# vineetbansal/scarlet

Hardware: AMD Instinct MI355X
Metric: PGM iters/sec on 10k 5-band 64x64 scenes (higher is better)
Workload: dtype f32

## Files before the change

include/scarlet_hip.h:

```cpp
#ifndef SCARLET_HIP_H
#define SCARLET_HIP_H

#include <stdint.h>

#ifdef __cplusplus
extern "C" {
#endif

#define SCARLET_OK            0
#define SCARLET_E_ARG        -1
#define SCARLET_E_TOO_LARGE  -2
#define SCARLET_E_HIP        -3
#define SCARLET_E_NOTIMPL    -4

#define SCARLET_MAX_SIDE     1024
#define SCARLET_MAX_COMPONENTS 256
#define SCARLET_MAX_OBSERVATIONS 8

#define SCARLET_FLAG_SED_NOT_CONVERGED   1
#define SCARLET_FLAG_MORPH_NOT_CONVERGED 2
#define SCARLET_FLAG_EDGE_PIXELS         4
#define SCARLET_FLAG_NO_VALID_PIXELS     8

#define SCARLET_STATUS_CENTER_AT_EDGE    1
#define SCARLET_STATUS_NONFINITE         2
#define SCARLET_STATUS_BAD_COUNT         4
#define SCARLET_STATUS_BAD_INIT          8

#define SCARLET_INIT_EXTENDED 0
#define SCARLET_INIT_POINT    1
#define SCARLET_MAX_LAYERS    8

#define SCARLET_SYM_KSPACE 0
#define SCARLET_SYM_SOFT   1
#define SCARLET_SYM_SDSS   2
#define SCARLET_SYM_FULL_WINDOW 16

#define SCARLET_NORM_SED       0
#define SCARLET_NORM_MORPH     1
#define SCARLET_NORM_MORPH_MAX 2

const char *scarlet_version(void);
const char *scarlet_last_error(void);
int scarlet_set_option(const char *name, int value);
int64_t scarlet_debug_stamps(int64_t *out, int64_t capacity);
int scarlet_next_fast_len(int n);


int scarlet_host_prox_monotonic_f64(double *x, int n, const int *ref_idx,
                                    const int *dist_idx, int n_dist, double thresh);

int scarlet_host_prox_weighted_monotonic_f32(float *x, int n, const float *weights,
                                             const int *offsets, const int *dist_idx,
                                             int n_dist, float thresh);
int scarlet_host_prox_weighted_monotonic_f64(double *x, int n, const double *weights,
                                             const int *offsets, const int *dist_idx,
                                             int n_dist, double thresh);

int scarlet_host_apply_filter_f32(const float *image, int H, int W, const float *values,
                                  const int *y_start, const int *y_end, const int *x_start,
                                  const int *x_end, int n, float *result);
int scarlet_host_apply_filter_f64(const double *image, int H, int W, const double *values,
                                  const int *y_start, const int *y_end, const int *x_start,
                                  const int *x_end, int n, double *result);


int scarlet_prox_weighted_monotonic(float *x, int n, int H, int W, const int32_t *centers,
                                    float thresh, void *stream);

int scarlet_prox_nearest_monotonic(float *x, int n, int H, int W, const int32_t *centers,
                                   float thresh, void *stream);

int scarlet_prox_symmetry(float *x, int n, int H, int W, const int32_t *centers,
                          const double *shifts, int algorithm, float strength,
                          int use_fill, float fill, void *stream);

int scarlet_max_pixel(const float *x, int n, int H, int W, int32_t *centers_io,
                      int32_t *status, void *stream);

int scarlet_psf_weighted_centroid(const float *x, int n, int H, int W, const double *psf,
                                  int P, int32_t *centers_io, double *shifts_out,
                                  int32_t *status, void *stream);

int scarlet_prox_plus(float *x, int64_t count, void *stream);
int scarlet_prox_hard(float *x, int64_t count, float thresh_times_step, void *stream);
int scarlet_prox_soft(float *x, int64_t count, float thresh_times_step, void *stream);

int scarlet_normalize(float *sed, float *morph, int n, int B, int HW, int type, void *stream);

int scarlet_log_range(const float *x, int n, int64_t count, double *out, void *stream);
int scarlet_log_hist(const float *x, int n, int64_t count, const double *edges,
                     const int32_t *nbins, int32_t *hist, void *stream);
int scarlet_cut_below(float *x, int64_t count, double thresh, void *stream);
int scarlet_trim(const float *x, int n, int H, int W, float min_value, int32_t *box, void *stream);
int scarlet_resample(const float *in, float *out, int n, int H, int W, const double *taps,
                     const int32_t *win0, int ny, int nx, void *stream);

int scarlet_apply_filter(const float *image, int H, int W, const float *values,
// ... 111 lines not shown
```

scarlet_amd/_lib.py:

```python
import ctypes
import os
from ctypes import (POINTER, Structure, c_char_p, c_double, c_float, c_int, c_int32, c_int64,
                    c_uint8, c_void_p)

HERE = os.path.dirname(os.path.abspath(__file__))
LIB_PATH = os.path.join(HERE, "csrc", "libscarlet_hip.so")
if os.environ.get("SCARLET_LIB_PATH"):
    LIB_PATH = os.environ["SCARLET_LIB_PATH"]


class HipLibraryMissing(ImportError):
    pass


if not os.path.exists(LIB_PATH):
    raise HipLibraryMissing(
        "scarlet_amd: {} not found.  The engine has no CPU fallback; build the HIP "
        "library first (make -C scarlet_amd/csrc).".format(LIB_PATH))

import torch

lib = ctypes.CDLL(LIB_PATH)

OK, E_ARG, E_TOO_LARGE, E_HIP, E_NOTIMPL = 0, -1, -2, -3, -4
FLAG_SED_NOT_CONVERGED, FLAG_MORPH_NOT_CONVERGED, FLAG_EDGE_PIXELS, FLAG_NO_VALID_PIXELS = 1, 2, 4, 8
STATUS_CENTER_AT_EDGE, STATUS_NONFINITE, STATUS_BAD_COUNT, STATUS_BAD_INIT = 1, 2, 4, 8
INIT_EXTENDED, INIT_POINT = 0, 1
MAX_LAYERS = 8
SYM_KSPACE, SYM_SOFT, SYM_SDSS = 0, 1, 2
SYM_FULL_WINDOW = 16
NORM_SED, NORM_MORPH, NORM_MORPH_MAX = 0, 1, 2
MAX_SIDE, MAX_COMPONENTS = 1024, 256
MAX_OBSERVATIONS = 8


class ScarletBatch(Structure):
    _fields_ = [
        ("S", c_int32), ("K", c_int32), ("B", c_int32), ("H", c_int32), ("W", c_int32),
        ("images", c_void_p), ("weights", c_void_p), ("weight_scalar", c_float),
        ("sed", c_void_p * 2), ("morph", c_void_p * 2), ("cur", c_void_p),
        ("centers", c_void_p), ("shifts", c_void_p), ("flags", c_void_p),
        ("fix_sed", c_void_p), ("fix_morph", c_void_p),
        ("lipschitz", c_void_p), ("mse", c_void_p), ("mse_capacity", c_int32),
        ("it", c_void_p), ("active", c_void_p), ("status", c_void_p),
        ("symmetric", c_int32), ("monotonic", c_int32),
        ("l0_thresh", c_float), ("l1_thresh", c_float),
        ("centroid_psf", c_void_p), ("centroid_P", c_int32),
        ("diff_kernel", c_void_p), ("psf_h", c_int32), ("psf_w", c_int32),
        ("diff_kernel_per_scene", c_int32),
        ("workspace", c_void_p),
        ("group", c_void_p),
        ("n_components", c_void_p),
    ]


class ScarletInitSpec(Structure):
    _fields_ = [
        ("bg_rms", c_void_p), ("bg_rms_per_scene", c_int32),
        ("obs_psf_peak", c_void_p), ("obs_psf_peak_per_scene", c_int32),
        ("model_psf", c_void_p), ("model_psf_P", c_int32),
        ("kind", c_void_p),
        ("flux_percentiles", c_void_p),
        ("thresh", c_float),
        ("init_symmetric", c_int32), ("init_monotonic", c_int32), ("run_update", c_int32),
    ]


class ScarletPrior(Structure):
    _fields_ = [
        ("grad_sed", c_void_p), ("grad_morph", c_void_p), ("L_sed", c_void_p), ("L_morph", c_void_p),
        ("quad_sed_weight", c_void_p), ("quad_sed_target", c_void_p),
        ("quad_morph_weight", c_void_p), ("quad_morph_target", c_void_p),
        ("L_comp", c_void_p),
    ]


_P = c_void_p
_SIGNATURES = {
    "scarlet_version": (c_char_p, []),
    "scarlet_last_error": (c_char_p, []),
    "scarlet_set_option": (c_int, [c_char_p, c_int]),
    "scarlet_debug_stamps": (c_int64, [_P, c_int64]),
    "scarlet_next_fast_len": (c_int, [c_int]),
    "scarlet_host_prox_monotonic_f64": (c_int, [_P, c_int, _P, _P, c_int, c_double]),
    "scarlet_host_prox_weighted_monotonic_f32": (c_int, [_P, c_int, _P, _P, _P, c_int, c_float]),
    "scarlet_host_prox_weighted_monotonic_f64": (c_int, [_P, c_int, _P, _P, _P, c_int, c_double]),
    "scarlet_host_apply_filter_f32": (c_int, [_P, c_int, c_int, _P, _P, _P, _P, _P, c_int, _P]),
    "scarlet_host_apply_filter_f64": (c_int, [_P, c_int, c_int, _P, _P, _P, _P, _P, c_int, _P]),
    "scarlet_prox_weighted_monotonic": (c_int, [_P, c_int, c_int, c_int, _P, c_float, _P]),
    "scarlet_prox_nearest_monotonic": (c_int, [_P, c_int, c_int, c_int, _P, c_float, _P]),
    "scarlet_prox_symmetry": (c_int, [_P, c_int, c_int, c_int, _P, _P, c_int, c_float, c_int, c_float, _P]),
    "scarlet_max_pixel": (c_int, [_P, c_int, c_int, c_int, _P, _P, _P]),
    "scarlet_psf_weighted_centroid": (c_int, [_P, c_int, c_int, c_int, _P, c_int, _P, _P, _P, _P]),
    "scarlet_match_psfs": (c_int, [_P, c_int, c_int, c_int, _P, c_int, c_int, c_int, _P, _P]),
    "scarlet_prox_plus": (c_int, [_P, c_int64, _P]),
    "scarlet_prox_hard": (c_int, [_P, c_int64, c_float, _P]),
    "scarlet_prox_soft": (c_int, [_P, c_int64, c_float, _P]),
    "scarlet_normalize": (c_int, [_P, _P, c_int, c_int, c_int, c_int, _P]),
    "scarlet_log_range": (c_int, [_P, c_int, c_int64, _P, _P]),
    "scarlet_log_hist": (c_int, [_P, c_int, c_int64, _P, _P, _P, _P]),
    "scarlet_cut_below": (c_int, [_P, c_int64, c_double, _P]),
    "scarlet_trim": (c_int, [_P, c_int, c_int, c_int, c_float, _P, _P]),
    "scarlet_resample": (c_int, [_P, _P, c_int, c_int, c_int, _P, _P, c_int, c_int, _P]),
    "scarlet_apply_filter": (c_int, [_P, c_int, c_int, _P, _P, _P, _P, _P, c_int, _P, _P]),
    "scarlet_batch_workspace_bytes": (c_int64, [POINTER(ScarletBatch)]),
    "scarlet_batch_pipelines": (c_int, [POINTER(ScarletBatch)]),
    "scarlet_fit": (c_int, [POINTER(ScarletBatch), c_int, c_double, c_int, c_int, _P]),
    "scarlet_fit_observations": (c_int, [POINTER(ScarletBatch), POINTER(POINTER(ScarletBatch)), _P, c_int, c_int, c_double, c_int, c_int, _P]),
    "scarlet_init_combined_sed": (c_int, [POINTER(ScarletBatch), _P, c_int, c_int, _P, c_int, _P, _P]),
    "scarlet_fit_multi": (c_int, [POINTER(ScarletBatch), POINTER(POINTER(ScarletBatch)), _P, c_int, c_int, c_double, c_int, c_int, _P]),
    "scarlet_backward_step": (c_int, [POINTER(ScarletBatch), c_int, _P]),
    "scarlet_backward_step_prior": (c_int, [POINTER(ScarletBatch), POINTER(ScarletPrior), c_int, _P]),
    "scarlet_source_update_prior": (c_int, [POINTER(ScarletBatch), POINTER(ScarletPrior), c_int, _P]),
    "scarlet_fit_prior": (c_int, [POINTER(ScarletBatch), POINTER(ScarletPrior), c_int, c_double, c_int, c_int, _P]),
    "scarlet_backward_gradients": (c_int, [POINTER(ScarletBatch), c_int, _P]),
    "scarlet_source_update": (c_int, [POINTER(ScarletBatch), c_int, _P]),
    "scarlet_check_convergence": (c_int, [POINTER(ScarletBatch), c_double, _P]),
    "scarlet_debug_psf_stamps_offset": (c_int64, [_P]),
    "scarlet_debug_psf_plan": (c_int, [_P, _P]),
    "scarlet_profile_begin": (c_int, [c_int]),
    "scarlet_profile_end": (c_int, [_P, _P]),
    "scarlet_profile_end_ex": (c_int, [_P, _P, _P]),
    "scarlet_init_extended": (c_int, [POINTER(ScarletBatch), _P, c_float, _P, c_int, c_int, c_int, _P]),
    "scarlet_init_sources": (c_int, [POINTER(ScarletBatch), POINTER(ScarletInitSpec), _P]),
    "scarlet_convergence_sums": (c_int, [POINTER(ScarletBatch), _P]),
    "scarlet_batch_prepare_psf": (c_int, [POINTER(ScarletBatch), _P]),
    "scarlet_convolve_same": (c_int, [_P, c_int, c_int, c_int, _P, c_int, c_int, c_int, _P, _P]),
}

EXPORTS = tuple(_SIGNATURES)

for _name, (_res, _args) in _SIGNATURES.items():
    _fn = getattr(lib, _name)
    _fn.restype = _res
    _fn.argtypes = _args
# ... 39 lines not shown
```

scarlet_amd/csrc/fused2.h:

```cpp
#pragma once
#include "fused.h"

#define SC_FB2 512
#define SC_NW2 (SC_FB2 / SC_WAVE)
#define SC_PAIR_VEC_FLOATS 512

struct KsLengths {
    unsigned short v[2][32];
    static constexpr int fast_len(int n)
    {
        for (int m = n;; ++m) {
            int q = m;
            while (q % 2 == 0) q /= 2;
            while (q % 3 == 0) q /= 3;
            while (q % 5 == 0) q /= 5;
            if (q == 1) return m;
        }
    }
    constexpr KsLengths() : v{}
    {
        for (int r = 0; r < 32; ++r) {
            const int F = fast_len(2 * (2 * r + 1) + 10);
            int Fe = F;
            while (Fe & 1) Fe = fast_len(Fe + 1);
            v[0][r] = (unsigned short)F; v[1][r] = (unsigned short)Fe;
        }
    }
};
__device__ const KsLengths sc_ks_lengths = KsLengths();
__device__ __forceinline__ unsigned ks_request_lengths(int tid)
{
    return tid < 64 ? (unsigned)(&sc_ks_lengths.v[0][0])[tid] : 0u;
}
__device__ __forceinline__ void ks_fill_lengths(unsigned short (*fl)[32], int tid, unsigned requested)
{
    if (tid < 64) (&fl[0][0])[tid] = (unsigned short)requested;
}
__device__ __forceinline__ KsGeom ks_geom(const SymWindow &s, const unsigned short (*fl)[32])
{
    KsGeom g;
    g.h = s.h; g.w = s.w; g.ry = s.h / 2; g.rx = s.w / 2;
    g.ntr = round16(s.h) >> 4; g.wp = round16(s.w); g.ntc = g.wp >> 4;
    g.Fy = uniform((int)fl[0][g.ry]);
    g.Fx = uniform((int)fl[1][g.rx]);
    return g;
}

template <int KM, int BM, int XS, bool P>
__device__ __forceinline__ int iterate2_body(const FusedArgs &a, const int s, const int c0, const int it_old, const bool resident,
                                             const bool reentered = false)
{
    static_assert(KM <= 4, "one pair of waves per component");
    static_assert(1 + KM * BM <= 32 && 4 * SC_NW2 == 32, "the partial sums are combined by 32 rows of 16 lanes");
    constexpr bool X = XS > 0;
    extern __shared__ __align__(16) float lds[];
    const int K = X ? KM : a.K, B = X ? BM : a.B, H = X ? XS : a.H, W = X ? XS : a.W, HW = H * W, LW = X ? SC_XS_STRIDE : tile_stride(W);
    const int tile_floats = H * LW;
#ifndef SC_TILE_B128
#define SC_TILE_B128 1
#endif
    auto tl4 = [](const float *p) {
        if constexpr (X && SC_TILE_B128 && (SC_XS_STRIDE % 4) == 0) return *reinterpret_cast<const float4 *>(p);
        else return lds_load4(p);
    };
    auto ts4 = [](float *p, float4 v) {
        if constexpr (X && SC_TILE_B128 && (SC_XS_STRIDE % 4) == 0) *reinterpret_cast<float4 *>(p) = v;
        else lds_store4(p, v);
    };
    const bool symmetric = X ? true : a.symmetric != 0, monotonic = X ? true : a.monotonic != 0;
    float *tiles = lds;
    float *vecs = lds + (size_t)K * tile_floats;
    constexpr int NG = KM * (KM + 1) / 2;
    constexpr int NP = 1 + KM * BM;
    constexpr int GPT = 2;
    constexpr int GPW = 8;
    __shared__ float red[4 * SC_NW2][NP > NG ? NP : NG];
    __shared__ double mat[2][KM * KM > BM * BM ? KM * KM : BM * BM];
    __shared__ float sed_s[KM * BM], sed_new[KM * BM];
    __shared__ float step_s[2];
    __shared__ double conv_s[KM][2], conv_m[KM][2][2];
    __shared__ int lstop_s[KM];
    __shared__ float nmax_s[KM][2];
    __shared__ int pair_flag[KM][2];
    __shared__ int arrive_s;
    __shared__ double cent_s[KM][2][3];
    __shared__ unsigned short fl_s[2][32];
    __shared__ int ctl_s[2][2];
    __shared__ int carry_cen[KM][2];
    __shared__ double carry_sh[KM][2];
    __shared__ float carry_sed[KM * BM];
    __shared__ short rowrange_s[KM][2][2];
    __shared__ unsigned place_s;
    const int tid = threadIdx.x, lane = tid & 63, wid = uniform(tid >> 6);
    float *const morph0 = a.morph[0], *const morph1 = a.morph[1], *const sed0 = a.sed[0], *const sed1 = a.sed[1];
    const float *min_g = (c0 ? morph1 : morph0) + (size_t)s * K * HW;
    float *mout_g = (c0 ? morph0 : morph1) + (size_t)s * K * HW;
    const float *sed_in = (c0 ? sed1 : sed0) + (size_t)s * K * B;
    float *sed_out = (c0 ? sed0 : sed1) + (size_t)s * K * B;
    const int it_new = it_old + 1;
    const int ngroups = HW >> 2, gpr = W >> 2;
    const float *img = a.images + (size_t)s * B * HW;
    const float *wgt = (!X && a.weights) ? a.weights + (size_t)s * B * HW : nullptr;
#define STAMP(i) do { if (a.stamps && tid == 0) a.stamps[(size_t)s * 16 + (i)] = (long long)__builtin_amdgcn_s_memtime(); } while (0)
#ifdef SC_STAMP_WORKER
#define WSTAMP(i) do { if (a.stamps && lane == 0) a.stamps[(size_t)s * 16 + 12 + (i)] = (long long)__builtin_amdgcn_s_memtime(); } while (0)
#else
#define WSTAMP(i) do { } while (0)
#endif
#ifdef SC_STAMP_PAIRS
    long long pst[3] = {0, 0, 0};
#define PSTAMP(i) do { if (a.stamps) pst[i] = (long long)__builtin_amdgcn_s_memtime(); } while (0)
#else
#define PSTAMP(i) do { } while (0)
#endif
    STAMP(0);
    if (a.stamps && tid == 0) a.stamps[(size_t)s * 16 + 7] = (long long)__builtin_amdgcn_s_memrealtime();
#ifdef SC_STAMP_PERIOD
    if (P && a.stamps && tid == 0) a.stamps[(size_t)a.S * 16 + (size_t)s * 2 + (it_new & 1)] = (long long)__builtin_amdgcn_s_memrealtime();
#endif
    if (P && a.stamps && tid == 0 && !reentered) {
        a.stamps[(size_t)s * 16 + 14] = (long long)__builtin_amdgcn_s_memrealtime();
        a.stamps[(size_t)s * 16 + 15] = (long long)__builtin_amdgcn_s_getreg(4 | (0 << 6) | (31 << 11))
                                        | ((long long)__builtin_amdgcn_s_getreg(20 | (0 << 6) | (31 << 11)) << 32);
    }
    const unsigned fl_req = ks_request_lengths(tid);
    const int n_present = a.ncomp ? scene_ncomp(a.ncomp, s, K) : K;
    const int slot = wid >> 1;
    int kp = slot;
    if constexpr (X) {
        unsigned place = 0x03020100u;
        if (P) { const unsigned lp = place_s; if (reentered) place = (unsigned)uniform((int)lp); }
        if (!(P && reentered) && !a.no_place) {
            int cost[KM];
#pragma unroll
            for (int j = 0; j < KM; ++j) {
                const int ccy = uniform(a.centers[2 * (s * K + j)]), ccx = uniform(a.centers[2 * (s * K + j) + 1]);
                const SymWindow w = sym_window(H, W, ccy, ccx);
                const int ntr = round16(w.h) >> 4, ntc = round16(w.w) >> 4;
                cost[j] = (j < n_present && !w.centered) ? ntr * ntc * (ntr + ntc) : 0;
            }
            place = 0;
#pragma unroll
            for (int j = 0; j < KM; ++j) {
                int rank = 0;
#pragma unroll
                for (int i = 0; i < KM; ++i) rank += (cost[i] > cost[j] || (cost[i] == cost[j] && i < j)) ? 1 : 0;
                place |= (unsigned)j << (8 * (rank ^ (rank >> 1)));
            }
        }
        if (P && !reentered && tid == 0) place_s = place;
        kp = (int)((place >> (8 * slot)) & (KM - 1));
    }
    int pre_cy = 0, pre_cx = 0;
    double pre_dy = 0, pre_dx = 0;
    if (X && kp < K) {
        const int cpre = s * K + kp;
        if (!(P && reentered)) {
            pre_cy = a.centers[2 * cpre]; pre_cx = a.centers[2 * cpre + 1];
            pre_dy = a.shifts[2 * cpre]; pre_dx = a.shifts[2 * cpre + 1];
        }
        if (P) {
            const int lcy = carry_cen[kp][0], lcx = carry_cen[kp][1];
            const double ldy = carry_sh[kp][0], ldx = carry_sh[kp][1];
            if (reentered) { pre_cy = lcy; pre_cx = lcx; pre_dy = ldy; pre_dx = ldx; }
        }
    }
    float *kcache = nullptr;
// ... 556 lines not shown
        q[0] = pst[2];
        q[1] = ((pst[2] - pst[1]) & 0xfffff) | (((pst[1] - pst[0]) & 0xfffff) << 20) | ((long long)(ls < 255 ? ls : 255) << 40) |
               ((long long)kg.ntr << 48) | ((long long)kg.ntc << 51) | ((long long)slot << 54);
    }
#endif
    __syncthreads();
    if (mine && norm == norm) {
        const double n2 = conv_m[k][0][1] + conv_m[k][1][1];
        if (n2 != n2) {
            norm = __builtin_nanf("");
            float4 *out4 = reinterpret_cast<float4 *>(mout_g + (size_t)k * HW);
            const float4 nan4 = make_float4(norm, norm, norm, norm);
            for (int g = g0; g < ngroups; g += 2 * SC_WAVE) out4[g] = nan4;
            if (lead && lane < B) { sed_out[k * B + lane] = norm; if (P) carry_sed[k * BM + lane] = norm; }
            if (P && lane == 0) {
                ctl_s[it_old & 1][1] = 0;
                rowrange_s[k][1 - c0][0] = 0; rowrange_s[k][1 - c0][1] = (short)(H - 1);
            }
        }
    }
    if (mine && lead && lane == 0) {
        if (!(norm > 0.f) || isinf(norm)) stat |= SCARLET_STATUS_NONFINITE;
        if (stat) atomicOr(&a.status[s], stat);
    }
    STAMP(5);

    if (wid == 0) {
        bool pending = false;
        if (lane < n_present && it_new > 1) {
            const int kk = lane;
            int set = 0;
            const double d2 = conv_m[kk][0][0] + conv_m[kk][1][0], n2 = conv_m[kk][0][1] + conv_m[kk][1][1];
            if (!(n2 == n2 && conv_s[kk][0] <= a.e_rel2 * conv_s[kk][1])) set |= SCARLET_FLAG_SED_NOT_CONVERGED;
            if (!(d2 <= a.e_rel2 * n2)) set |= SCARLET_FLAG_MORPH_NOT_CONVERGED;
            const int clear = (SCARLET_FLAG_SED_NOT_CONVERGED | SCARLET_FLAG_MORPH_NOT_CONVERGED) & ~set;
            if (clear) atomicAnd(&a.flags[s * K + kk], ~clear);
            if (set) atomicOr(&a.flags[s * K + kk], set);
            pending = set != 0;
        }
        const bool done = it_new > 1 && __builtin_amdgcn_ballot_w64(pending) == 0;
        if (lane == 0) {
            a.it[s] = it_new;
            a.cur[s] = 1 - c0;
            if (done) { a.active[s] = 0; if (P) ctl_s[it_old & 1][0] = 0; }
        }
    }
    STAMP(6);
    if (a.stamps && tid == 0) a.stamps[(size_t)s * 16 + 11] = (long long)__builtin_amdgcn_s_memrealtime();
#undef STAMP
#undef WSTAMP
#undef PSTAMP
    if (P) {
        __syncthreads();
        return uniform(ctl_s[it_old & 1][0] | (ctl_s[it_old & 1][1] << 1));
    }
    return 0;
}

template <int KM, int BM, int XS = 0>
__global__ __launch_bounds__(SC_FB2, 4) void k_iterate2(FusedArgs a)
{
    const int s = blockIdx.x;
    const int active_s = a.active[s], c0 = a.cur[s], it_old = a.it[s];
    asm volatile("" ::"s"(c0), "s"(it_old));
    if (!active_s) return;
    iterate2_body<KM, BM, XS, false>(a, s, c0, it_old, false);
}

#define SC_FIT2X_KERNEL k_fit2x
#define SC_FIT2X_REENTER(scene, state, it)                                                                     \
    asm volatile("s_mov_b64 exec, -1\n\t"                                                                      \
                 "s_mov_b64 s[0:1], %0\n\t"                                                                    \
                 "s_mov_b32 s2, %1\n\t"                                                                        \
                 "s_mov_b32 s3, %2\n\t"                                                                        \
                 "s_mov_b32 s4, %3\n\t"                                                                        \
                 "v_mov_b32 v0, %4\n\t"                                                                        \
                 "s_getpc_b64 s[6:7]\n\t"                                                                      \
                 "s_add_u32 s6, s6, k_fit2x@rel32@lo+4\n\t"                                                    \
                 "s_addc_u32 s7, s7, k_fit2x@rel32@hi+12\n\t"                                                  \
                 "s_waitcnt lgkmcnt(0)\n\t"                                                                    \
                 "s_setpc_b64 s[6:7]"                                                                          \
                 :                                                                                             \
                 : "s"(__builtin_amdgcn_kernarg_segment_ptr()), "s"(scene), "s"(state), "s"(it), "v"((int)threadIdx.x) \
                 : "s0", "s1", "s2", "s3", "s4", "s6", "s7", "v0", "scc", "memory")
extern "C" __global__ __launch_bounds__(SC_FB2, 4) void SC_FIT2X_KERNEL(FusedArgs a, int n_iter, int *queue, int n_workgroups)
{
    const int s = blockIdx.x;
    const unsigned st = (unsigned)__builtin_amdgcn_workgroup_id_y();
    int c0 = 0, it = 0, left = 0;
    bool resident = false, run = true;
    if (st >> 31) {
        resident = ((st >> 30) & 1) && !(n_iter & (1 << 30));
        c0 = (int)((st >> 29) & 1); left = (int)(st & 0x1fffffffu);
        it = (int)__builtin_amdgcn_workgroup_id_z();
    } else {
        const int active_s = a.active[s];
        c0 = a.cur[s]; it = a.it[s];
        asm volatile("" ::"s"(c0), "s"(it));
        left = n_iter & 0xffffff;
        run = active_s && left > 0;
    }
    if (run) {
        const int r = iterate2_body<4, 5, 64, true>(a, s, c0, it, resident, (st >> 31) != 0);
        if ((r & 1) && left > 1) {
            const unsigned nst = 0x80000000u | ((unsigned)(r >> 1) << 30) | ((unsigned)(c0 ^ 1) << 29) | (unsigned)(left - 1);
            if (!(r & 2) || (n_iter & (1 << 30))) {
                asm volatile("s_waitcnt vmcnt(0)" ::: "memory");
                __syncthreads();
            }
            SC_FIT2X_REENTER(s, nst, it + 1);
        }
    }
    __shared__ int next_s;
    if (threadIdx.x == 0) next_s = queue ? atomicAdd(queue, 1) + n_workgroups : a.S;
    __syncthreads();
    const int nx = uniform(next_s);
    __syncthreads();
    if (nx < a.S) SC_FIT2X_REENTER(nx, 0u, 0);
}
```

scarlet_amd/csrc/scarlet_hip.hip:

```cpp
#include <hip/hip_runtime.h>
#include <math.h>
#include <stdio.h>
#include <string.h>
#include <stdlib.h>
#include <atomic>
#include <map>
#include <mutex>
#include <tuple>
#include <vector>
#include <algorithm>
#include <hipfft/hipfft.h>

#include "common.h"
#include "prox_ops.h"
#include "engine.h"
#include "fused.h"
#include "fused2.h"
#include "bigk.h"
#include "hugek.h"
#include "boxupdate.h"
#include "psf_path.h"
#include "fftconv.h"
#include "extras.h"
#include "initsrc.h"
#include "multiobs.h"
#include "prior.h"

__constant__ unsigned short sc_nfl_table[SC_NFL_MAX];

static thread_local char g_err[512] = "";
static int set_err(int code, const char *msg)
{
    snprintf(g_err, sizeof(g_err), "%s", msg);
    return code;
}
#define HIP_TRY(expr)                                                                    \
    do {                                                                                 \
        hipError_t e_ = (expr);                                                          \
        if (e_ != hipSuccess) {                                                          \
            snprintf(g_err, sizeof(g_err), "%s failed: %s (%s:%d)", #expr,               \
                     hipGetErrorString(e_), __FILE__, __LINE__);                         \
            return SCARLET_E_HIP;                                                        \
        }                                                                                \
    } while (0)

extern "C" const char *scarlet_version(void) { return "scarlet_amd-hip 0.2 (gfx950)"; }

enum { OPT_NO_EXACT = 0, OPT_NO_KSCACHE, OPT_FUSED_V1, OPT_NO_FUSED, OPT_FORCE_BLOCK_UPDATE, OPT_NO_HYBRID_SWEEP,
       OPT_PAD_LDS, OPT_STAMPS, OPT_PSF_HIPFFT, OPT_NO_BOX, OPT_NO_BOX2, OPT_NO_PSF3PASS, OPT_NO_SIDE_STREAM, OPT_NO_GRAM_MFMA, OPT_NO_BIGK_FUSED, OPT_NO_PIPELINE, OPT_NO_PERSIST, OPT_PERSIST_DBG, OPT_FORCE_HUGEK, OPT_NO_PLACE, OPT_COUNT };
static const char *const g_opt_names[OPT_COUNT] = {"NO_EXACT", "NO_KSCACHE", "FUSED_V1", "NO_FUSED", "FORCE_BLOCK_UPDATE",
                                                   "NO_HYBRID_SWEEP", "PAD_LDS", "STAMPS", "PSF_HIPFFT", "NO_BOX", "NO_BOX2",
                                                   "NO_PSF3PASS", "NO_SIDE_STREAM", "NO_GRAM_MFMA", "NO_BIGK_FUSED", "NO_PIPELINE", "NO_PERSIST", "PERSIST_DBG", "FORCE_HUGEK", "NO_PLACE"};
static std::atomic<int> g_opt[OPT_COUNT];
static std::once_flag g_opt_once;
static void options_init(void)
{
    std::call_once(g_opt_once, [] {
        for (int i = 0; i < OPT_COUNT; ++i) {
            char name[64];
            snprintf(name, sizeof(name), "SCARLET_%s", g_opt_names[i]);
            const char *v = getenv(name);
            int val = 0;
            if (v) { val = atoi(v); if (val == 0 && v[0] != '0') val = 1; }
            if (v && !v[0]) val = 1;
            g_opt[i].store(val, std::memory_order_relaxed);
        }
    });
}
static inline int opt(int which) { options_init(); return g_opt[which].load(std::memory_order_relaxed); }
static std::atomic<bool> g_layout_frozen{false};
static std::atomic<bool> g_hugek_frozen{false};
extern "C" int scarlet_set_option(const char *name, int value)
{
    options_init();
    if (!name) return set_err(SCARLET_E_ARG, "null option name");
    for (int i = 0; i < OPT_COUNT; ++i)
        if (!strcmp(name, g_opt_names[i])) {
            if (i == OPT_FORCE_HUGEK && g_hugek_frozen.load() && (g_opt[i].load() != 0) != (value != 0))
                return set_err(SCARLET_E_ARG, "FORCE_HUGEK fixes the workspace layout of batches with 8 < K <= 32: it cannot "
                                              "change after the first such workspace of the process was sized");
            if ((i == OPT_PSF_HIPFFT || i == OPT_STAMPS) && g_layout_frozen.load() && (g_opt[i].load() != 0) != (value != 0))
                return set_err(SCARLET_E_ARG, "PSF_HIPFFT / STAMPS fix the workspace layout of PSF batches: they cannot change "
                                              "after the first PSF workspace of the process was sized");
            return g_opt[i].exchange(value) != 0 ? 1 : 0;
        }
    return set_err(SCARLET_E_ARG, "unknown option");
}

struct DevBuf {
    void *p = nullptr;
    ~DevBuf() { if (p) (void)hipFree(p); }
    DevBuf() = default;
    DevBuf(const DevBuf &) = delete;
    DevBuf &operator=(const DevBuf &) = delete;
    template <typename T> T *as() const { return (T *)p; }
};
#define DEV_ALLOC(buf, bytes) HIP_TRY(hipMalloc(&(buf).p, (bytes)))
extern "C" const char *scarlet_last_error(void) { return g_err; }

extern "C" int scarlet_next_fast_len(int n)
{
    if (n <= 1) return 1;
    long best = -1;
    for (long p5 = 1; p5 < 2L * n; p5 *= 5)
        for (long p35 = p5; p35 < 2L * n; p35 *= 3) {
// ... 1488 lines not shown
        u.gscratch = ws_at<float>(b, l.gscratch);
        const size_t lds = sizeof(float) * (2 * round16(b->H) + 5 * round16(b->W) +
                                            stage_floats(round16(b->H), round16(b->W)));
        if ((rc = allow_lds(k_source_update<2>, lds))) return rc;
        hipLaunchKernelGGL(k_source_update<2>, dim3(b->S * b->K), dim3(SC_BLOCK), lds, (hipStream_t)stream, u);
    }
    HIP_TRY(hipGetLastError());
    return SCARLET_OK;
}

extern "C" int scarlet_source_update(scarlet_batch *b, int in_iteration, void *stream)
{
    int rc = check_batch(b);
    if (!rc) rc = check_counts(b, stream);
    if (rc) return rc;
    return launch_update(b, ws_layout(b, WS_PEEK), in_iteration ? 1 : 0, in_iteration ? 0 : 1, stream);
}

static int launch_converge(scarlet_batch *b, const WsLayout &l, double e_rel, void *stream)
{
    hipLaunchKernelGGL(k_converge, dim3((b->S + SC_BLOCK - 1) / SC_BLOCK), dim3(SC_BLOCK), 0, (hipStream_t)stream,
                       b->S, b->K, ws_at<double>(b, l.conv), b->flags, b->active, b->it, b->cur, e_rel * e_rel,
                       (const int *)b->n_components);
    HIP_TRY(hipGetLastError());
    return SCARLET_OK;
}
extern "C" int scarlet_check_convergence(scarlet_batch *b, double e_rel, void *stream)
{
    int rc = check_batch(b);
    if (!rc) rc = check_counts(b, stream);
    return rc ? rc : launch_converge(b, ws_layout(b, WS_PEEK), e_rel, stream);
}

static int fit2x_resident_workgroups(size_t lds, int *out)
{
    static std::mutex mu;
    static int cached[64] = {0};
    static size_t cached_lds[64] = {0};
    int dev = 0;
    HIP_TRY(hipGetDevice(&dev));
    if (dev < 0 || dev >= 64) return set_err(SCARLET_E_HIP, "device index out of range");
    std::lock_guard<std::mutex> lock(mu);
    if (!cached[dev] || cached_lds[dev] != lds) {
        int per_cu = 0, cus = 0;
        HIP_TRY(hipOccupancyMaxActiveBlocksPerMultiprocessor(&per_cu, k_fit2x, SC_FB2, lds));
        HIP_TRY(hipDeviceGetAttribute(&cus, hipDeviceAttributeMultiprocessorCount, dev));
        if (per_cu < 1) per_cu = 1;
        cached[dev] = per_cu * cus; cached_lds[dev] = lds;
    }
    *out = cached[dev];
    return SCARLET_OK;
}

static size_t fused_lds_bytes(const scarlet_batch *b)
{
    return sizeof(float) * ((size_t)b->K * b->H * tile_stride(b->W) + SC_NWAVES * SC_WAVE_VEC_FLOATS);
}
static bool fused_ok(const scarlet_batch *b, int approximate_L)
{
    if (approximate_L || b->diff_kernel || b->K > 4 || b->group || opt(OPT_NO_FUSED)) return false;
    if (b->H > 64 || b->W > 64 || (b->W & 3) || b->H < 3 || b->W < 3) return false;
    return fused_lds_bytes(b) <= LDS_LIMIT - 4096;
}
static int launch_fused(scarlet_batch *b, const WsLayout &l, double e_rel, void *stream, int n_iter, int *done)
{
    if (done) *done = 1;
    int rc = ensure_tables();
    if (rc) return rc;
    FusedArgs f;
    f.S = b->S; f.K = b->K; f.B = b->B; f.H = b->H; f.W = b->W;
    f.images = b->images; f.weights = b->weights; f.weight_scalar = b->weight_scalar;
    f.sed[0] = b->sed[0]; f.sed[1] = b->sed[1]; f.morph[0] = b->morph[0]; f.morph[1] = b->morph[1];
    f.cur = b->cur; f.fix_sed = b->fix_sed; f.fix_morph = b->fix_morph;
    f.centers = b->centers; f.shifts = b->shifts; f.flags = b->flags;
    f.lipschitz = b->lipschitz; f.mse = b->mse; f.mse_capacity = b->mse_capacity;
    f.it = b->it; f.active = b->active; f.status = b->status;
    f.symmetric = b->symmetric; f.monotonic = b->monotonic; f.l0_thresh = b->l0_thresh; f.l1_thresh = b->l1_thresh;
    f.centroid_psf = b->centroid_psf; f.centroid_P = b->centroid_P; f.e_rel2 = e_rel * e_rel;
    f.ncomp = b->n_components;
    f.no_place = opt(OPT_NO_PLACE) != 0;
    f.kscache = (!l.has_kscache || b->diff_kernel || opt(OPT_NO_KSCACHE)) ? nullptr : ws_at<float>(b, l.kscache);
    f.stamps = (opt(OPT_STAMPS) && n_partials(b->K, b->B) >= 16) ? ws_at<long long>(b, l.partials) : nullptr;
    const size_t lds = fused_lds_bytes(b) + (size_t)opt(OPT_PAD_LDS);
    hipStream_t st = (hipStream_t)stream;
#define LAUNCH_ITERATE(KM_, BM_)                                                                       \
    do {                                                                                               \
        rc = allow_lds(k_iterate<KM_, BM_>, lds);                                                      \
        if (rc) return rc;                                                                             \
        prof_start(4, st);                                                                             \
        hipLaunchKernelGGL((k_iterate<KM_, BM_>), dim3(b->S), dim3(SC_BLOCK), lds, st, f);             \
        prof_stop(st);                                                                                 \
    } while (0)
    if (b->K <= 4 && b->B <= 5 && !opt(OPT_FUSED_V1)) {
        const size_t lds2 = sizeof(float) * ((size_t)b->K * b->H * tile_stride(b->W) + (size_t)b->K * SC_PAIR_VEC_FLOATS) +
                            (size_t)opt(OPT_PAD_LDS);
#define LAUNCH_ITERATE2(BM_)                                                                           \
    do {                                                                                               \
        rc = allow_lds(k_iterate2<4, BM_>, lds2);                                                      \
        if (rc) return rc;                                                                             \
        prof_start(4, st);                                                                             \
        hipLaunchKernelGGL((k_iterate2<4, BM_>), dim3(b->S), dim3(SC_FB2), lds2, st, f);               \
        prof_stop(st);                                                                                 \
    } while (0)
        const bool exact64 = b->K == 4 && b->B == 5 && b->H == 64 && b->W == 64 && !b->weights && b->weight_scalar == 1.0f && b->symmetric &&
                             b->monotonic && b->l0_thresh < 0.f && b->l1_thresh < 0.f && !opt(OPT_NO_EXACT);
        const size_t lds2x = sizeof(float) * ((size_t)4 * 64 * SC_XS_STRIDE + (size_t)4 * SC_PAIR_VEC_FLOATS) + (size_t)opt(OPT_PAD_LDS);
        if (n_iter > 0xffffff) n_iter = 0xffffff;
        if (exact64 && (n_iter > 1 || (opt(OPT_PERSIST_DBG) & 2)) && !opt(OPT_NO_PERSIST)) {
            rc = allow_lds(k_fit2x, lds2x);
            if (rc) return rc;
            int n_wg = 0;
            if ((rc = fit2x_resident_workgroups(lds2x, &n_wg))) return rc;
            if (n_wg > b->S || (opt(OPT_PERSIST_DBG) & 4)) n_wg = b->S;
            int *queue = ws_at<int>(b, l.fit2x_queue);
            HIP_TRY(hipMemsetAsync(queue, 0, sizeof(int), st));
            prof_start(4, st, n_iter);
            hipLaunchKernelGGL(k_fit2x, dim3(n_wg), dim3(SC_FB2), lds2x, st, f, n_iter | ((opt(OPT_PERSIST_DBG) & 1) << 30), queue, n_wg);
            prof_stop(st);
            if (done) *done = n_iter;
        } else if (exact64) {
            rc = allow_lds(k_iterate2<4, 5, 64>, lds2x);
            if (rc) return rc;
            prof_start(4, st);
            hipLaunchKernelGGL((k_iterate2<4, 5, 64>), dim3(b->S), dim3(SC_FB2), lds2x, st, f);
            prof_stop(st);
        } else
            LAUNCH_ITERATE2(5);
#undef LAUNCH_ITERATE2
        HIP_TRY(hipGetLastError());
        return SCARLET_OK;
    }
    if (b->B <= 6) LAUNCH_ITERATE(4, 6); else LAUNCH_ITERATE(4, SC_BMAX);
#undef LAUNCH_ITERATE
    HIP_TRY(hipGetLastError());
    return SCARLET_OK;
}

__global__ void k_count_active(const int *active, int S, int *out)
{
    int c = 0;
    for (int i = threadIdx.x; i < S; i += blockDim.x) c += active[i] != 0;
    c = (int)wave_sum((float)c);
    __shared__ int tot;
    if (threadIdx.x == 0) tot = 0;
    __syncthreads();
    if ((threadIdx.x & 63) == 0) atomicAdd(&tot, c);
    __syncthreads();
    if (threadIdx.x == 0) *out = tot;
}

extern "C" int scarlet_fit(scarlet_batch *b, int max_iter, double e_rel, int approximate_L,
                           int check_every, void *stream)
{
    int rc = check_batch(b);
    if (rc) return rc;
    if (max_iter < 0) return set_err(SCARLET_E_ARG, "max_iter < 0");
    if ((rc = check_counts(b, stream))) return rc;
    hipStream_t st = (hipStream_t)stream;
    int launched = 0;
    const WsLayout l = ws_layout(b, WS_FIX);
    int *d_count = ws_at<int>(b, l.active_count);
    const bool fused = fused_ok(b, approximate_L);
    if (!fused && two_pipelines(l)) {
        SideStream *side = nullptr;
        if ((rc = side_stream(&side))) return rc;
        if (side) {
            scarlet_batch v[2];
            WsLayout lv[2];
            split_views(b, l, v, lv);
            hipStream_t sv[2] = {st, side->st};
// ... 570 lines not shown
```

Measured before the change: 16.66 million.

## Split tail scenes into iteration laps to balance persistent fit2x workgroups

Adds a lap-based schedule to the persistent fit2x kernel. The last T scenes (by default twice the resident workgroup count) are split into chunks of a few iterations each, and a work unit waits through a device-scope progress counter until the previous lap of its scene finishes. The aim is to cut tail imbalance, where a few workgroups finish long-running scenes while the rest sit idle. In exchange it adds global-memory handoff of centers, shifts and SEDs between laps, spin-polling with a timeout status flag, and a reset kernel launch.

```diff
diff --git a/include/scarlet_hip.h b/include/scarlet_hip.h
--- a/include/scarlet_hip.h
+++ b/include/scarlet_hip.h
@@ -26,6 +26,7 @@
 #define SCARLET_STATUS_NONFINITE         2
 #define SCARLET_STATUS_BAD_COUNT         4
 #define SCARLET_STATUS_BAD_INIT          8
+#define SCARLET_STATUS_LAP_TIMEOUT      16
 
 #define SCARLET_INIT_EXTENDED 0
 #define SCARLET_INIT_POINT    1
@@ -44,6 +45,8 @@
 const char *scarlet_last_error(void);
 int scarlet_set_option(const char *name, int value);
 int64_t scarlet_debug_stamps(int64_t *out, int64_t capacity);
+int64_t scarlet_debug_fit2x_plan(int S, int n_wg, int n_iter, int T, int c, int32_t *out, int64_t capacity, int32_t *out4);
+int scarlet_debug_fit2x_launch_plan(int S, int n_iter, int32_t *out5);
 int scarlet_next_fast_len(int n);
 
 
diff --git a/scarlet_amd/_lib.py b/scarlet_amd/_lib.py
--- a/scarlet_amd/_lib.py
+++ b/scarlet_amd/_lib.py
@@ -25,6 +25,7 @@
 OK, E_ARG, E_TOO_LARGE, E_HIP, E_NOTIMPL = 0, -1, -2, -3, -4
 FLAG_SED_NOT_CONVERGED, FLAG_MORPH_NOT_CONVERGED, FLAG_EDGE_PIXELS, FLAG_NO_VALID_PIXELS = 1, 2, 4, 8
 STATUS_CENTER_AT_EDGE, STATUS_NONFINITE, STATUS_BAD_COUNT, STATUS_BAD_INIT = 1, 2, 4, 8
+STATUS_LAP_TIMEOUT = 16
 INIT_EXTENDED, INIT_POINT = 0, 1
 MAX_LAYERS = 8
 SYM_KSPACE, SYM_SOFT, SYM_SDSS = 0, 1, 2
@@ -81,6 +82,8 @@
     "scarlet_last_error": (c_char_p, []),
     "scarlet_set_option": (c_int, [c_char_p, c_int]),
     "scarlet_debug_stamps": (c_int64, [_P, c_int64]),
+    "scarlet_debug_fit2x_plan": (c_int64, [c_int, c_int, c_int, c_int, c_int, _P, c_int64, _P]),
+    "scarlet_debug_fit2x_launch_plan": (c_int, [c_int, c_int, _P]),
     "scarlet_next_fast_len": (c_int, [c_int]),
     "scarlet_host_prox_monotonic_f64": (c_int, [_P, c_int, _P, _P, c_int, c_double]),
     "scarlet_host_prox_weighted_monotonic_f32": (c_int, [_P, c_int, _P, _P, _P, c_int, c_float]),
diff --git a/scarlet_amd/csrc/fit2x_plan.h b/scarlet_amd/csrc/fit2x_plan.h
--- /dev/null
+++ b/scarlet_amd/csrc/fit2x_plan.h
@@ -0,0 +1,54 @@
+#pragma once
+
+#if defined(__HIPCC__) || defined(__CUDACC__)
+#define SC_PLAN_FN __host__ __device__ inline
+#else
+#define SC_PLAN_FN static inline
+#endif
+
+#define SC_LAP_ITERS_DEFAULT 5
+#define SC_LAP_SCENES_PER_WG 2
+
+struct Fit2xPlan {
+    int tail;
+    int chunk;
+    int laps;
+    int units;
+};
+struct Fit2xUnit {
+    int scene, lap, first, count, last;
+    int pos;
+};
+
+SC_PLAN_FN Fit2xPlan fit2x_plan(int S, int n_wg, int n_iter, int T_req, int c_req)
+{
+    Fit2xPlan p;
+    p.chunk = c_req > 0 ? c_req : SC_LAP_ITERS_DEFAULT;
+    long long T = T_req < 0 ? (long long)SC_LAP_SCENES_PER_WG * (n_wg > 0 ? n_wg : 0) : T_req;
+    if (T > S) T = S;
+    if (S <= n_wg || n_iter <= p.chunk) T = 0;
+    if (T && (((long long)(n_iter - 1) / p.chunk + 1) * T + S > 0x3fffffffLL || (n_iter - 1) / p.chunk + 1 > 0x7fffff)) T = 0;
+    p.tail = (int)T;
+    p.laps = p.tail ? (n_iter - 1) / p.chunk + 1 : 1;
+    p.units = S - p.tail + p.laps * p.tail;
+    return p;
+}
+
+SC_PLAN_FN Fit2xUnit fit2x_unit(int S, int n_iter, int T, int c, int u)
+{
+    Fit2xUnit r;
+    const int head = S - T;
+    if (u < head || T <= 0) {
+        r.scene = u; r.lap = 0; r.first = 0; r.count = n_iter; r.last = 1; r.pos = -1;
+        return r;
+    }
+    const int v = u - head;
+    r.lap = v / T;
+    r.pos = v - r.lap * T;
+    r.scene = head + r.pos;
+    r.first = r.lap * c;
+    const int end = n_iter - r.first < c ? n_iter : r.first + c;
+    r.count = end - r.first;
+    r.last = end >= n_iter;
+    return r;
+}
diff --git a/scarlet_amd/csrc/fused2.h b/scarlet_amd/csrc/fused2.h
--- a/scarlet_amd/csrc/fused2.h
+++ b/scarlet_amd/csrc/fused2.h
@@ -1,5 +1,6 @@
 #pragma once
 #include "fused.h"
+#include "fit2x_plan.h"
 
 #define SC_FB2 512
 #define SC_NW2 (SC_FB2 / SC_WAVE)
@@ -48,7 +49,7 @@
 
 template <int KM, int BM, int XS, bool P>
 __device__ __forceinline__ int iterate2_body(const FusedArgs &a, const int s, const int c0, const int it_old, const bool resident,
-                                             const bool reentered = false)
+                                             const bool reentered = false, const unsigned cont = 0)
 {
     static_assert(KM <= 4, "one pair of waves per component");
     static_assert(1 + KM * BM <= 32 && 4 * SC_NW2 == 32, "the partial sums are combined by 32 rows of 16 lanes");
@@ -113,6 +114,24 @@
 #else
 #define PSTAMP(i) do { } while (0)
 #endif
+    if (P && cont) {
+        auto dev_load = [](const auto *p) { return __hip_atomic_load(p, __ATOMIC_RELAXED, __HIP_MEMORY_SCOPE_AGENT); };
+        const int j = tid & 63;
+        if (wid == 0 && j < 2 * K) carry_cen[j >> 1][j & 1] = dev_load(a.centers + 2 * (s * K + (j >> 1)) + (j & 1));
+        if (wid == 1 && j < 2 * K)
+            carry_sh[j >> 1][j & 1] = __longlong_as_double(
+                dev_load(reinterpret_cast<const long long *>(a.shifts) + 2 * (s * K + (j >> 1)) + (j & 1)));
+        if (wid == 2 && j < K * B)
+            carry_sed[(j / B) * BM + (j % B)] = __int_as_float(dev_load(reinterpret_cast<const int *>(sed_in) + j));
+        if (wid == 3 && j < KM * 4) (&rowrange_s[0][0][0])[j] = (short)((j & 1) ? H - 1 : 0);
+        if (wid == 4 && j == 0) {
+            unsigned pl = 0;
+#pragma unroll
+            for (int q = 0; q < KM; ++q) pl |= ((cont >> (2 * q)) & 3u) << (8 * q);
+            place_s = pl;
+        }
+        __syncthreads();
+    }
     STAMP(0);
     if (a.stamps && tid == 0) a.stamps[(size_t)s * 16 + 7] = (long long)__builtin_amdgcn_s_memrealtime();
 #ifdef SC_STAMP_PERIOD
@@ -775,7 +794,9 @@
 #undef PSTAMP
     if (P) {
         __syncthreads();
-        return uniform(ctl_s[it_old & 1][0] | (ctl_s[it_old & 1][1] << 1));
+        const unsigned pl = place_s;
+        return uniform(ctl_s[it_old & 1][0] | (ctl_s[it_old & 1][1] << 1) |
+                       (int)((((pl >> 0) & 3u) | ((pl >> 6) & 0xcu) | ((pl >> 12) & 0x30u) | ((pl >> 18) & 0xc0u)) << 8));
     }
     return 0;
 }
@@ -806,38 +827,87 @@
                  :                                                                                             \
                  : "s"(__builtin_amdgcn_kernarg_segment_ptr()), "s"(scene), "s"(state), "s"(it), "v"((int)threadIdx.x) \
                  : "s0", "s1", "s2", "s3", "s4", "s6", "s7", "v0", "scc", "memory")
-extern "C" __global__ __launch_bounds__(SC_FB2, 4) void SC_FIT2X_KERNEL(FusedArgs a, int n_iter, int *queue, int n_workgroups)
+__device__ __forceinline__ int *fit2x_scratch()
 {
-    const int s = blockIdx.x;
+    extern __shared__ __align__(16) float lds[];
+    return reinterpret_cast<int *>(lds + 4 * 64 * SC_XS_STRIDE);
+}
+#define SC_LAP_WORD(laps, place8) ((int)(((unsigned)(place8) << 24) | (unsigned)(laps)))
+#define SC_LAP_COUNT 0x7fffff
+#define SC_LAP_VOID 0x800000
+#define SC_LAP_POLLS (1 << 22)
+extern "C" __global__ __launch_bounds__(SC_FB2, 4) void SC_FIT2X_KERNEL(FusedArgs a, int n_iter, int *queue, int n_workgroups,
+                                                                        int *progress, int lap_scenes, int lap_iters, int n_units)
+{
+    __shared__ int next_s;
+    int *const scratch = fit2x_scratch();
+    int s = blockIdx.x;
     const unsigned st = (unsigned)__builtin_amdgcn_workgroup_id_y();
     int c0 = 0, it = 0, left = 0;
-    bool resident = false, run = true;
+    unsigned cont = 0, place8 = 0xe4u;
+    bool resident = false, run = true, lap_void = false;
     if (st >> 31) {
         resident = ((st >> 30) & 1) && !(n_iter & (1 << 30));
-        c0 = (int)((st >> 29) & 1); left = (int)(st & 0x1fffffffu);
+        c0 = (int)((st >> 29) & 1); left = (int)(st & 0xffffffu);
         it = (int)__builtin_amdgcn_workgroup_id_z();
     } else {
-        const int active_s = a.active[s];
-        c0 = a.cur[s]; it = a.it[s];
-        asm volatile("" ::"s"(c0), "s"(it));
-        left = n_iter & 0xffffff;
-        run = active_s && left > 0;
+        const Fit2xUnit un = fit2x_unit(a.S, n_iter & 0xffffff, lap_scenes, lap_iters, s);
+        if (threadIdx.x == 0) next_s = s;
+        __syncthreads();
+        s = un.scene;
+        left = un.count;
+        if (un.lap == 0) {
+            const int active_s = a.active[s];
+            c0 = a.cur[s]; it = a.it[s];
+            asm volatile("" ::"s"(c0), "s"(it));
+            run = active_s && left > 0;
+        } else {
+            if (threadIdx.x == 0) {
+                int w = 0, polls = 0;
+                while (((w = __hip_atomic_load(progress + un.pos, __ATOMIC_RELAXED, __HIP_MEMORY_SCOPE_AGENT)) & SC_LAP_COUNT) < un.lap) {
+                    if (++polls > SC_LAP_POLLS) break;
+                    __builtin_amdgcn_s_sleep(16);
+                }
+                __builtin_amdgcn_fence(__ATOMIC_ACQUIRE, "agent");
+                scratch[0] = w;
+            }
+            __syncthreads();
+            const int w = uniform(scratch[0]);
+            place8 = (w & SC_LAP_COUNT) ? (unsigned)w >> 24 : 0xe4u;
+            const int active_s = uniform(__hip_atomic_load(a.active + s, __ATOMIC_RELAXED, __HIP_MEMORY_SCOPE_AGENT));
+            c0 = uniform(__hip_atomic_load(a.cur + s, __ATOMIC_RELAXED, __HIP_MEMORY_SCOPE_AGENT));
+            it = uniform(__hip_atomic_load(a.it + s, __ATOMIC_RELAXED, __HIP_MEMORY_SCOPE_AGENT));
+            const bool late = (w & SC_LAP_COUNT) < un.lap;
+            if (late && threadIdx.x == 0) atomicOr(&a.status[s], SCARLET_STATUS_LAP_TIMEOUT);
+            lap_void = late || (w & SC_LAP_VOID);
+            run = active_s && !lap_void;
+            cont = 0x100u | place8;
+        }
     }
     if (run) {
-        const int r = iterate2_body<4, 5, 64, true>(a, s, c0, it, resident, (st >> 31) != 0);
+        const int r = iterate2_body<4, 5, 64, true>(a, s, c0, it, resident, (st >> 31) != 0 || cont != 0, cont);
         if ((r & 1) && left > 1) {
-            const unsigned nst = 0x80000000u | ((unsigned)(r >> 1) << 30) | ((unsigned)(c0 ^ 1) << 29) | (unsigned)(left - 1);
+            const unsigned nst = 0x80000000u | ((unsigned)((r >> 1) & 1) << 30) | ((unsigned)(c0 ^ 1) << 29) | (unsigned)(left - 1);
             if (!(r & 2) || (n_iter & (1 << 30))) {
                 asm volatile("s_waitcnt vmcnt(0)" ::: "memory");
                 __syncthreads();
             }
             SC_FIT2X_REENTER(s, nst, it + 1);
         }
-    }
-    __shared__ int next_s;
-    if (threadIdx.x == 0) next_s = queue ? atomicAdd(queue, 1) + n_workgroups : a.S;
+        place8 = ((unsigned)r >> 8) & 0xffu;
+    }
+    {
+        const Fit2xUnit un = fit2x_unit(a.S, n_iter & 0xffffff, lap_scenes, lap_iters, uniform(next_s));
+        if (un.pos >= 0 && !un.last) {
+            asm volatile("s_waitcnt vmcnt(0)" ::: "memory");
+            __syncthreads();
+            if (threadIdx.x == 0)
+                __hip_atomic_store(progress + un.pos, SC_LAP_WORD((un.lap + 1) | (lap_void ? SC_LAP_VOID : 0), place8), __ATOMIC_RELEASE, __HIP_MEMORY_SCOPE_AGENT);
+        }
+    }
+    __syncthreads();
+    if (threadIdx.x == 0) next_s = queue ? atomicAdd(queue, 1) + n_workgroups : n_units;
     __syncthreads();
     const int nx = uniform(next_s);
-    __syncthreads();
-    if (nx < a.S) SC_FIT2X_REENTER(nx, 0u, 0);
+    if (nx < n_units) SC_FIT2X_REENTER(nx, 0u, 0);
 }
diff --git a/scarlet_amd/csrc/scarlet_hip.hip b/scarlet_amd/csrc/scarlet_hip.hip
--- a/scarlet_amd/csrc/scarlet_hip.hip
+++ b/scarlet_amd/csrc/scarlet_hip.hip
@@ -47,10 +47,12 @@
 extern "C" const char *scarlet_version(void) { return "scarlet_amd-hip 0.2 (gfx950)"; }
 
 enum { OPT_NO_EXACT = 0, OPT_NO_KSCACHE, OPT_FUSED_V1, OPT_NO_FUSED, OPT_FORCE_BLOCK_UPDATE, OPT_NO_HYBRID_SWEEP,
-       OPT_PAD_LDS, OPT_STAMPS, OPT_PSF_HIPFFT, OPT_NO_BOX, OPT_NO_BOX2, OPT_NO_PSF3PASS, OPT_NO_SIDE_STREAM, OPT_NO_GRAM_MFMA, OPT_NO_BIGK_FUSED, OPT_NO_PIPELINE, OPT_NO_PERSIST, OPT_PERSIST_DBG, OPT_FORCE_HUGEK, OPT_NO_PLACE, OPT_COUNT };
+       OPT_PAD_LDS, OPT_STAMPS, OPT_PSF_HIPFFT, OPT_NO_BOX, OPT_NO_BOX2, OPT_NO_PSF3PASS, OPT_NO_SIDE_STREAM, OPT_NO_GRAM_MFMA, OPT_NO_BIGK_FUSED, OPT_NO_PIPELINE, OPT_NO_PERSIST, OPT_PERSIST_DBG, OPT_FORCE_HUGEK, OPT_NO_PLACE,
+       OPT_NO_LAPS, OPT_LAP_ITERS, OPT_LAP_SCENES, OPT_FIT2X_WG, OPT_COUNT };
 static const char *const g_opt_names[OPT_COUNT] = {"NO_EXACT", "NO_KSCACHE", "FUSED_V1", "NO_FUSED", "FORCE_BLOCK_UPDATE",
                                                    "NO_HYBRID_SWEEP", "PAD_LDS", "STAMPS", "PSF_HIPFFT", "NO_BOX", "NO_BOX2",
-                                                   "NO_PSF3PASS", "NO_SIDE_STREAM", "NO_GRAM_MFMA", "NO_BIGK_FUSED", "NO_PIPELINE", "NO_PERSIST", "PERSIST_DBG", "FORCE_HUGEK", "NO_PLACE"};
+                                                   "NO_PSF3PASS", "NO_SIDE_STREAM", "NO_GRAM_MFMA", "NO_BIGK_FUSED", "NO_PIPELINE", "NO_PERSIST", "PERSIST_DBG", "FORCE_HUGEK", "NO_PLACE",
+                                                   "NO_LAPS", "LAP_ITERS", "LAP_SCENES", "FIT2X_WG"};
 static std::atomic<int> g_opt[OPT_COUNT];
 static std::once_flag g_opt_once;
 static void options_init(void)
@@ -1645,6 +1647,53 @@
     return SCARLET_OK;
 }
 
+static Fit2xPlan fit2x_launch_plan(int S, int n_wg, int n_iter)
+{
+    const int T = opt(OPT_NO_LAPS) ? 0 : opt(OPT_LAP_SCENES) > 0 ? opt(OPT_LAP_SCENES) : -1;
+    return fit2x_plan(S, n_wg, n_iter, T, opt(OPT_LAP_ITERS));
+}
+static size_t fit2x_lds_bytes(void)
+{
+    return sizeof(float) * ((size_t)4 * 64 * SC_XS_STRIDE + (size_t)4 * SC_PAIR_VEC_FLOATS) + (size_t)opt(OPT_PAD_LDS);
+}
+static int fit2x_launch_workgroups(int S, size_t lds, int *out)
+{
+    int n_wg = 0, rc = fit2x_resident_workgroups(lds, &n_wg);
+    if (rc) return rc;
+    if (opt(OPT_FIT2X_WG) > 0 && n_wg > opt(OPT_FIT2X_WG)) n_wg = opt(OPT_FIT2X_WG);
+    if (n_wg > S || (opt(OPT_PERSIST_DBG) & 4)) n_wg = S;
+    *out = n_wg;
+    return SCARLET_OK;
+}
+extern "C" int scarlet_debug_fit2x_launch_plan(int S, int n_iter, int32_t *out5)
+{
+    if (S < 1 || n_iter < 1 || n_iter > 0xffffff || !out5)
+        return set_err(SCARLET_E_ARG, "scarlet_debug_fit2x_launch_plan: S >= 1, 1 <= n_iter <= 0xffffff, out5 != NULL");
+    int n_wg = 0, rc = fit2x_launch_workgroups(S, fit2x_lds_bytes(), &n_wg);
+    if (rc) return rc;
+    const Fit2xPlan p = fit2x_launch_plan(S, n_wg, n_iter);
+    out5[0] = p.tail; out5[1] = p.chunk; out5[2] = p.laps; out5[3] = p.units; out5[4] = n_wg;
+    return SCARLET_OK;
+}
+extern "C" int64_t scarlet_debug_fit2x_plan(int S, int n_wg, int n_iter, int T, int c, int32_t *out, int64_t capacity, int32_t *out4)
+{
+    if (S < 1 || n_wg < 1 || n_iter < 1 || n_iter > 0xffffff || (out && capacity < 0))
+        return set_err(SCARLET_E_ARG, "scarlet_debug_fit2x_plan: S, n_wg >= 1 and 1 <= n_iter <= 0xffffff");
+    const Fit2xPlan p = fit2x_plan(S, n_wg, n_iter, T, c);
+    if (out4) { out4[0] = p.tail; out4[1] = p.chunk; out4[2] = p.laps; out4[3] = p.units; }
+    for (int64_t u = 0; out && u < p.units && u < capacity; ++u) {
+        const Fit2xUnit un = fit2x_unit(S, n_iter, p.tail, p.chunk, (int)u);
+        out[4 * u] = un.scene; out[4 * u + 1] = un.lap; out[4 * u + 2] = un.first; out[4 * u + 3] = un.count;
+    }
+    return p.units;
+}
+__global__ void k_fit2x_reset(int *queue, int *progress, int n)
+{
+    const int i = blockIdx.x * blockDim.x + threadIdx.x;
+    if (i == 0) *queue = 0;
+    if (i < n) progress[i] = 0;
+}
+
 static size_t fused_lds_bytes(const scarlet_batch *b)
 {
     return sizeof(float) * ((size_t)b->K * b->H * tile_stride(b->W) + SC_NWAVES * SC_WAVE_VEC_FLOATS);
@@ -1697,18 +1746,19 @@
     } while (0)
         const bool exact64 = b->K == 4 && b->B == 5 && b->H == 64 && b->W == 64 && !b->weights && b->weight_scalar == 1.0f && b->symmetric &&
                              b->monotonic && b->l0_thresh < 0.f && b->l1_thresh < 0.f && !opt(OPT_NO_EXACT);
-        const size_t lds2x = sizeof(float) * ((size_t)4 * 64 * SC_XS_STRIDE + (size_t)4 * SC_PAIR_VEC_FLOATS) + (size_t)opt(OPT_PAD_LDS);
+        const size_t lds2x = fit2x_lds_bytes();
         if (n_iter > 0xffffff) n_iter = 0xffffff;
         if (exact64 && (n_iter > 1 || (opt(OPT_PERSIST_DBG) & 2)) && !opt(OPT_NO_PERSIST)) {
             rc = allow_lds(k_fit2x, lds2x);
             if (rc) return rc;
             int n_wg = 0;
-            if ((rc = fit2x_resident_workgroups(lds2x, &n_wg))) return rc;
-            if (n_wg > b->S || (opt(OPT_PERSIST_DBG) & 4)) n_wg = b->S;
-            int *queue = ws_at<int>(b, l.fit2x_queue);
-            HIP_TRY(hipMemsetAsync(queue, 0, sizeof(int), st));
+            if ((rc = fit2x_launch_workgroups(b->S, lds2x, &n_wg))) return rc;
+            const Fit2xPlan plan = fit2x_launch_plan(b->S, n_wg, n_iter);
+            int *queue = ws_at<int>(b, l.fit2x_queue), *progress = ws_at<int>(b, l.box_list);
+            hipLaunchKernelGGL(k_fit2x_reset, dim3((plan.tail + 256) / 256), dim3(256), 0, st, queue, progress, plan.tail);
             prof_start(4, st, n_iter);
-            hipLaunchKernelGGL(k_fit2x, dim3(n_wg), dim3(SC_FB2), lds2x, st, f, n_iter | ((opt(OPT_PERSIST_DBG) & 1) << 30), queue, n_wg);
+            hipLaunchKernelGGL(k_fit2x, dim3(n_wg), dim3(SC_FB2), lds2x, st, f, n_iter | ((opt(OPT_PERSIST_DBG) & 1) << 30), queue, n_wg,
+                               progress, plan.tail, plan.chunk, plan.units);
             prof_stop(st);
             if (done) *done = n_iter;
         } else if (exact64) {
```

After: 16.79 million (median of 6 runs). No clear change (+0.8%).
